# TorbenHellriegel/Speaker-Recognition-x-vectors

Hardware: AMD Instinct MI355X
Metric: x-vector embeddings/sec (300-frame utt) (higher is better)
Workload: dtype f32; 1 GPU; configs[1]: 1xMI355X batch=256 fixed 300-frame x 24-MFCC utterances, fp32 frame-level stack, extract_x_vec layer 6, random-init weights seed 42; build=xvec_hip gfx950 build 527c31bee3f9, batch_per_gpu=256, frames=300

## Files before the change

### speaker-recognition-x-vectors_amd/csrc/tdnn_wino_s3.hip

```cpp
#include "tdnn_wino_rows.h"

namespace xvec {
namespace wino {

constexpr int kS3K = 16;
constexpr int kS3Plane = kPairs * kS3K * 2;
constexpr int kS3Stage = 4 * 3 * kS3Plane;
constexpr int kS3Const = kConst * 4;
constexpr int kS3LdsBytes = 2 * kS3Stage + kS3Const + 2 * kTbl * 4 + 2 * 8;

__device__ __forceinline__ void s3_advance(const TdnnArgs& a, Ctx& cx, const Lane& ln, int* tbl, int64_t* tblh, int n_chunks) {
    if (cx.kc + 1 < n_chunks) {
        ++cx.kc;
    } else {
        const int64_t g_rem = cx.g_end - cx.g_s;
        const int64_t g_next = cx.g_s + (g_rem < 2 ? g_rem : 2);
        if (g_next < cx.g_end) {
            cx.g_s = g_next;
            cx.q0 = g_next * 32;
            cx.lp ^= 1;
            set_rows(a, cx, ln, tbl, tblh);
            cx.kc = 0;
        }
    }
}

struct S3Stage {
    float4 x0, x1, x2, x3;
};

__device__ __forceinline__ void s3_gld(const Ctx& cx, bool grp, S3Stage& s) {
    const int xo0 = grp ? cx.x01 : cx.x00, xo3 = grp ? cx.x31 : cx.x30;
    const int so = cx.kc * (kS3K * 4);
    s.x0 = buf_load16(cx.xrsrc, xo0, so);
    s.x1 = buf_load16(cx.xrsrc, xo0, so + cx.drb);
    s.x2 = buf_load16(cx.xrsrc, xo0, so + 2 * cx.drb);
    s.x3 = buf_load16(cx.xrsrc, xo3, so);
}

__device__ __forceinline__ void s3_vstore(char* B, int st, const S3Stage& s) {
    const float4 v[4] = {
        make_float4(s.x0.x - s.x2.x, s.x0.y - s.x2.y, s.x0.z - s.x2.z, s.x0.w - s.x2.w),
        make_float4(s.x1.x + s.x2.x, s.x1.y + s.x2.y, s.x1.z + s.x2.z, s.x1.w + s.x2.w),
        make_float4(s.x2.x - s.x1.x, s.x2.y - s.x1.y, s.x2.z - s.x1.z, s.x2.w - s.x1.w),
        make_float4(s.x1.x - s.x3.x, s.x1.y - s.x3.y, s.x1.z - s.x3.z, s.x1.w - s.x3.w)};
#pragma unroll
    for (int k = 0; k < 4; ++k) {
        u32x2 hi, mid, lo;
        split3(v[k], hi, mid, lo);
        *reinterpret_cast<u32x2*>(B + (3 * k + 0) * kS3Plane + st) = hi;
        *reinterpret_cast<u32x2*>(B + (3 * k + 1) * kS3Plane + st) = mid;
        *reinterpret_cast<u32x2*>(B + (3 * k + 2) * kS3Plane + st) = lo;
    }
}

__device__ __forceinline__ void s3_uld(__amdgpu_buffer_rsrc_t rsrc, int voff, float4* w, int k, int c, int n_chunks) {
    if (c >= n_chunks) c -= n_chunks;
#pragma unroll
    for (int p = 0; p < 3; ++p) w[p] = buf_load16(rsrc, voff, ((4 * c + k) * 3 + p) * 1024);
}

template <int G>
__device__ __forceinline__ void s3_tile(const TdnnArgs& a, char* lds, int* tbl, int64_t* tblh, Ctx& cx, const Lane& ln,
                                        S3Stage& st, float4 (&w)[4][3], __amdgpu_buffer_rsrc_t ursrc, int n0, int tp,
                                        int n_chunks) {
    const bool grp = (threadIdx.x >> 2) & 1;
    f32x16 acc0_0, acc0_1, acc1_0, acc1_1, acc2_0, acc2_1, acc3_0, acc3_1;
#pragma unroll
    for (int e = 0; e < 16; ++e) {
        acc0_0[e] = 0.f; acc1_0[e] = 0.f; acc2_0[e] = 0.f; acc3_0[e] = 0.f;
        acc0_1[e] = 0.f; acc1_1[e] = 0.f; acc2_1[e] = 0.f; acc3_1[e] = 0.f;
    }
    for (int it = 0; it < n_chunks; ++it) {
        const char* S = lds + (it & 1) * kS3Stage;
        char* Sn = lds + ((it & 1) ^ 1) * kS3Stage;
        s3_vstore(Sn, ln.st_off, st);
        s3_advance(a, cx, ln, tbl, tblh, n_chunks);
        s3_gld(cx, grp, st);
#define WS3_PRODUCT(K_)                                                                                        \
        {                                                                                                      \
            float4 xf0[3], xf1[3];                                                                             \
            _Pragma("unroll") for (int pl = 0; pl < 3; ++pl) {                                                 \
                xf0[pl] = *reinterpret_cast<const float4*>(S + (3 * K_ + pl) * kS3Plane + ln.a_rd);            \
                if constexpr (G > 1)                                                                           \
                    xf1[pl] = *reinterpret_cast<const float4*>(S + (3 * K_ + pl) * kS3Plane + 32 * 32 + ln.a_rd); \
            }                                                                                                  \
            s3_mfma6(acc##K_##_0, xf0, w[K_]);                                                                 \
            if constexpr (G > 1) s3_mfma6(acc##K_##_1, xf1, w[K_]);                                            \
            s3_uld(ursrc, ln.b_rd, w[K_], K_, it + 1, n_chunks);                                               \
        }
        WS3_PRODUCT(0) WS3_PRODUCT(1) WS3_PRODUCT(2) WS3_PRODUCT(3)
#undef WS3_PRODUCT
        __syncthreads();
    }

    epilogue<G>(a, reinterpret_cast<const float*>(lds + 2 * kS3Stage), tbl, tblh, ln, n0, tp, acc0_0, acc1_0, acc2_0, acc3_0, acc0_1,
                acc1_1, acc2_1, acc3_1);
}

__global__ __launch_bounds__(256, 2) void tdnn_wino_s3_kernel(const TdnnArgs a) {
    extern __shared__ __attribute__((aligned(16))) char lds[];
    float* cst = reinterpret_cast<float*>(lds + 2 * kS3Stage);
    int* tbl = reinterpret_cast<int*>(cst + kConst);
    int64_t* tblh = reinterpret_cast<int64_t*>(tbl + 2 * kTbl);
    Ctx cx;
    Lane ln;
    const int n0 = block_setup(a, 3, cx, ln);
    const int n_chunks = 2 * a.cpt;
    const int64_t g_begin = cx.g_s, g_end = cx.g_end;
    const int tid = threadIdx.x, lane = tid & 63, wave = ln.wave;
    ln.st_off = (ln.r0 + 32 * ((tid >> 2) & 1)) * (kS3K * 2) + (tid & 3) * 8;
    ln.a_rd = ln.r * (kS3K * 2) + ln.h * 16;
    ln.b_rd = lane * 16;
    ln.sw = 0;
    const int64_t ct = n0 / 32 + wave;
    const __amdgpu_buffer_rsrc_t ursrc = make_rsrc(static_cast<const char*>(a.Wf) + ct * (int64_t)n_chunks * 12288);

    stream_start(a, n0, cst, tbl, tblh, cx, ln);

    const bool grp = (tid >> 2) & 1;
    S3Stage st;
    float4 w[4][3];
    s3_gld(cx, grp, st);
#pragma unroll
    for (int k = 0; k < 4; ++k) s3_uld(ursrc, ln.b_rd, w[k], k, 0, n_chunks);
    s3_vstore(lds, ln.st_off, st);
    s3_advance(a, cx, ln, tbl, tblh, n_chunks);
    s3_gld(cx, grp, st);
    __syncthreads();

    int64_t g = g_begin;
    int tp = 0;
    for (; g + 2 <= g_end; g += 2, tp ^= 1) s3_tile<2>(a, lds, tbl, tblh, cx, ln, st, w, ursrc, n0, tp, n_chunks);
    if (g < g_end) s3_tile<1>(a, lds, tbl, tblh, cx, ln, st, w, ursrc, n0, tp, n_chunks);
}

}

bool tdnn_wino_s3_applicable(const TdnnGeom& g, int ldx) {
    return tdnn_wino_applicable(g, ldx) && (g.kpt_pad / wino::kS3K) % 2 == 0;
}

hipError_t launch_tdnn_wino_s3(const TdnnArgs& a, hipStream_t s) {
    if (a.groups_total <= 0 || a.blocks_per_col <= 0 || a.blocks_per_col > a.groups_total || a.tap_rows < 1 || a.cpt < 1 ||
        a.Wf == nullptr || (a.out_map.offsets == nullptr && a.p_fixed < 1))
        return hipErrorInvalidValue;
    const int grid = a.blocks_per_col * a.n_tiles;
    wino::tdnn_wino_s3_kernel<<<dim3(grid), dim3(256), wino::kS3LdsBytes, s>>>(a);
    return hipGetLastError();
}

}
```

Measured before the change: 151,400 embeddings/s.

## Software-pipeline S3 Winograd K-loop with interleaved LDS reads and swizzled LDS layout

Restructures the S3 Winograd TDNN inner loop so the MFMAs for each product are interleaved with LDS fragment reads for the next product and with weight buffer loads, using scheduling barriers. The next chunk's first fragments are prefetched across the __syncthreads. It also introduces an XOR-swizzled LDS address map for staging stores and fragment reads, aimed at avoiding bank conflicts. The intent is to hide LDS and global latency behind MFMA work, at the cost of more live registers and more complex control, including an extra barrier when n_chunks is 2.

```diff
diff --git a/profiles/diag/kloop_outline.py b/profiles/diag/kloop_outline.py
--- /dev/null
+++ b/profiles/diag/kloop_outline.py
@@ -0,0 +1,71 @@
+#!/usr/bin/env python3
+import re
+import sys
+
+KINDS = (("mfma", r"v_mfma_"), ("buffer_load", r"buffer_load_"), ("buffer_store", r"buffer_store_"), ("ds_read", r"ds_read"),
+         ("ds_write", r"ds_write"), ("s_barrier", r"s_barrier"), ("v_mov64", r"v_mov_b64|v_pk_mov_b32"),
+         ("branch", r"s_cbranch|s_branch"))
+
+
+def blocks(asm, kernel):
+    out, cur, inside = [], None, False
+    for line in asm.splitlines():
+        s = line.strip()
+        m = re.match(r"^([A-Za-z_.$][\w.$]*):", s)
+        if m:
+            lab = m.group(1)
+            if not lab.startswith(".L"):
+                inside = kernel in lab
+            if inside:
+                cur = (lab, [])
+                out.append(cur)
+            continue
+        if inside and cur is not None and s and not s.startswith((".", ";")):
+            cur[1].append(s.split(";")[0].strip())
+            if s.startswith("s_endpgm"):
+                inside = False
+    return out
+
+
+def kind_of(ins):
+    if ins.startswith("s_waitcnt"):
+        return ins
+    for k, pat in KINDS:
+        if re.match(pat, ins):
+            return k
+    return None
+
+
+def outline(instrs):
+    runs = []
+    for ins in instrs:
+        k = kind_of(ins)
+        if k is None:
+            continue
+        if runs and runs[-1][0] == k and not k.startswith("s_waitcnt"):
+            runs[-1][1] += 1
+        else:
+            runs.append([k, 1])
+    return [k if n == 1 else f"{k} x{n}" for k, n in runs]
+
+
+def main():
+    kernel = sys.argv[1]
+    min_mfma = int(sys.argv[2]) if len(sys.argv) > 2 else 12
+    asm = sys.stdin.read()
+    for lab, ins in blocks(asm, kernel):
+        if sum(1 for i in ins if i.startswith("v_mfma_")) < min_mfma:
+            continue
+        print(f"{lab}:  ({len(ins)} instructions)")
+        line = "   "
+        for item in outline(ins):
+            if len(line) + len(item) > 118:
+                print(line)
+                line = "   "
+            line += " " + item + " |"
+        print(line)
+        print()
+
+
+if __name__ == "__main__":
+    main()
diff --git a/speaker-recognition-x-vectors_amd/csrc/tdnn_wino_s3.hip b/speaker-recognition-x-vectors_amd/csrc/tdnn_wino_s3.hip
--- a/speaker-recognition-x-vectors_amd/csrc/tdnn_wino_s3.hip
+++ b/speaker-recognition-x-vectors_amd/csrc/tdnn_wino_s3.hip
@@ -1,11 +1,10 @@
 #include "tdnn_wino_rows.h"
+#include "wino_s3_lds_map.h"
 
 namespace xvec {
 namespace wino {
 
-constexpr int kS3K = 16;
-constexpr int kS3Plane = kPairs * kS3K * 2;
-constexpr int kS3Stage = 4 * 3 * kS3Plane;
+static_assert(kS3Pairs == kPairs, "wino_s3_lds_map.h: kS3K, kS3Plane, kS3Stage and the image of a (product, plane) block");
 constexpr int kS3Const = kConst * 4;
 constexpr int kS3LdsBytes = 2 * kS3Stage + kS3Const + 2 * kTbl * 4 + 2 * 8;
 
@@ -54,16 +53,54 @@
     }
 }
 
-__device__ __forceinline__ void s3_uld(__amdgpu_buffer_rsrc_t rsrc, int voff, float4* w, int k, int c, int n_chunks) {
-    if (c >= n_chunks) c -= n_chunks;
-#pragma unroll
-    for (int p = 0; p < 3; ++p) w[p] = buf_load16(rsrc, voff, ((4 * c + k) * 3 + p) * 1024);
-}
+struct S3U {
+    float4 w00, w01, w02, w10, w11, w12, w20, w21, w22, w30, w31, w32;
+};
+struct S3Frag {
+    float4 a0, a1, a2, b0, b1, b2;
+};
+
+#define WS3_MF(acc_, x_, w_) \
+    acc_ = __builtin_amdgcn_mfma_f32_32x32x16_bf16(__builtin_bit_cast(bf16x8, x_), __builtin_bit_cast(bf16x8, w_), acc_, 0, 0, 0);
+#define WS3_RD(dst_, B_, kn_, pl_, g_) \
+    dst_ = *reinterpret_cast<const float4*>((B_) + (3 * (kn_) + (pl_)) * kS3Plane + ((g_) ? a_rd1 : ln.a_rd));
+#define WS3_ULD(K_)                                                                   \
+    {                                                                                 \
+        int c_ = it + 1;                                                              \
+        if (c_ >= n_chunks) c_ -= n_chunks;                                           \
+        u.w##K_##0 = buf_load16(ursrc, ln.b_rd, ((4 * c_ + K_) * 3 + 0) * 1024);      \
+        u.w##K_##1 = buf_load16(ursrc, ln.b_rd, ((4 * c_ + K_) * 3 + 1) * 1024);      \
+        u.w##K_##2 = buf_load16(ursrc, ln.b_rd, ((4 * c_ + K_) * 3 + 2) * 1024);      \
+    }
+#define WS3_PRODUCT2(K_, NB_, kn_, BAR_)                                                                   \
+    {                                                                                                      \
+        WS3_MF(acc##K_##_0, f.a2, u.w##K_##0) WS3_RD(f.b2, S, K_, 2, 1) SB();                              \
+        WS3_MF(acc##K_##_0, f.a1, u.w##K_##1) WS3_RD(f.b1, S, K_, 1, 1) SB();                              \
+        WS3_MF(acc##K_##_0, f.a0, u.w##K_##2) WS3_RD(f.b0, S, K_, 0, 1) SB();                              \
+        WS3_MF(acc##K_##_0, f.a1, u.w##K_##0) WS3_MF(acc##K_##_0, f.a0, u.w##K_##1) WS3_MF(acc##K_##_0, f.a0, u.w##K_##0) SB(); \
+        BAR_                                                                                               \
+        WS3_MF(acc##K_##_1, f.b2, u.w##K_##0) WS3_RD(f.a2, NB_, kn_, 2, 0) SB();                           \
+        WS3_MF(acc##K_##_1, f.b1, u.w##K_##1) WS3_RD(f.a1, NB_, kn_, 1, 0) SB();                           \
+        WS3_MF(acc##K_##_1, f.b0, u.w##K_##2) WS3_RD(f.a0, NB_, kn_, 0, 0) SB();                           \
+        WS3_MF(acc##K_##_1, f.b1, u.w##K_##0) WS3_MF(acc##K_##_1, f.b0, u.w##K_##1) WS3_MF(acc##K_##_1, f.b0, u.w##K_##0) SB(); \
+        WS3_ULD(K_)                                                                                        \
+        SB();                                                                                              \
+    }
+#define WS3_PRODUCT1(K_, C_, N_, NB_, kn_, BAR_)                                                           \
+    {                                                                                                      \
+        BAR_                                                                                               \
+        WS3_MF(acc##K_##_0, f.C_##2, u.w##K_##0) WS3_RD(f.N_##2, NB_, kn_, 2, 0) SB();                     \
+        WS3_MF(acc##K_##_0, f.C_##1, u.w##K_##1) WS3_RD(f.N_##1, NB_, kn_, 1, 0) SB();                     \
+        WS3_MF(acc##K_##_0, f.C_##0, u.w##K_##2) WS3_RD(f.N_##0, NB_, kn_, 0, 0) SB();                     \
+        WS3_MF(acc##K_##_0, f.C_##1, u.w##K_##0) WS3_MF(acc##K_##_0, f.C_##0, u.w##K_##1) WS3_MF(acc##K_##_0, f.C_##0, u.w##K_##0) SB(); \
+        WS3_ULD(K_)                                                                                        \
+        SB();                                                                                              \
+    }
 
 template <int G>
 __device__ __forceinline__ void s3_tile(const TdnnArgs& a, char* lds, int* tbl, int64_t* tblh, Ctx& cx, const Lane& ln,
-                                        S3Stage& st, float4 (&w)[4][3], __amdgpu_buffer_rsrc_t ursrc, int n0, int tp,
-                                        int n_chunks) {
+                                        int a_rd1, S3Stage& st, S3U& u, S3Frag& f, __amdgpu_buffer_rsrc_t ursrc, int n0,
+                                        int tp, int n_chunks) {
     const bool grp = (threadIdx.x >> 2) & 1;
     f32x16 acc0_0, acc0_1, acc1_0, acc1_1, acc2_0, acc2_1, acc3_0, acc3_1;
 #pragma unroll
@@ -77,25 +114,23 @@
         s3_vstore(Sn, ln.st_off, st);
         s3_advance(a, cx, ln, tbl, tblh, n_chunks);
         s3_gld(cx, grp, st);
-#define WS3_PRODUCT(K_)                                                                                        \
-        {                                                                                                      \
-            float4 xf0[3], xf1[3];                                                                             \
-            _Pragma("unroll") for (int pl = 0; pl < 3; ++pl) {                                                 \
-                xf0[pl] = *reinterpret_cast<const float4*>(S + (3 * K_ + pl) * kS3Plane + ln.a_rd);            \
-                if constexpr (G > 1)                                                                           \
-                    xf1[pl] = *reinterpret_cast<const float4*>(S + (3 * K_ + pl) * kS3Plane + 32 * 32 + ln.a_rd); \
-            }                                                                                                  \
-            s3_mfma6(acc##K_##_0, xf0, w[K_]);                                                                 \
-            if constexpr (G > 1) s3_mfma6(acc##K_##_1, xf1, w[K_]);                                            \
-            s3_uld(ursrc, ln.b_rd, w[K_], K_, it + 1, n_chunks);                                               \
+        SB();
+        if constexpr (G > 1) {
+            WS3_PRODUCT2(0, S, 1, )
+            WS3_PRODUCT2(1, S, 2, )
+            WS3_PRODUCT2(2, S, 3, )
+            WS3_PRODUCT2(3, Sn, 0, __syncthreads(); SB();)
+        } else {
+            WS3_PRODUCT1(0, a, b, S, 1, )
+            WS3_PRODUCT1(1, b, a, S, 2, )
+            WS3_PRODUCT1(2, a, b, S, 3, )
+            WS3_PRODUCT1(3, b, a, Sn, 0, __syncthreads(); SB();)
         }
-        WS3_PRODUCT(0) WS3_PRODUCT(1) WS3_PRODUCT(2) WS3_PRODUCT(3)
-#undef WS3_PRODUCT
-        __syncthreads();
     }
 
     epilogue<G>(a, reinterpret_cast<const float*>(lds + 2 * kS3Stage), tbl, tblh, ln, n0, tp, acc0_0, acc1_0, acc2_0, acc3_0, acc0_1,
                 acc1_1, acc2_1, acc3_1);
+    if (n_chunks == 2) __syncthreads();
 }
 
 __global__ __launch_bounds__(256, 2) void tdnn_wino_s3_kernel(const TdnnArgs a) {
@@ -109,10 +144,11 @@
     const int n_chunks = 2 * a.cpt;
     const int64_t g_begin = cx.g_s, g_end = cx.g_end;
     const int tid = threadIdx.x, lane = tid & 63, wave = ln.wave;
-    ln.st_off = (ln.r0 + 32 * ((tid >> 2) & 1)) * (kS3K * 2) + (tid & 3) * 8;
-    ln.a_rd = ln.r * (kS3K * 2) + ln.h * 16;
+    ln.st_off = s3_st_off(tid);
+    ln.a_rd = s3_a_rd(lane, 0);
+    const int a_rd1 = s3_a_rd(lane, 1);
+    ln.sw = 0;
     ln.b_rd = lane * 16;
-    ln.sw = 0;
     const int64_t ct = n0 / 32 + wave;
     const __amdgpu_buffer_rsrc_t ursrc = make_rsrc(static_cast<const char*>(a.Wf) + ct * (int64_t)n_chunks * 12288);
 
@@ -120,20 +156,31 @@
 
     const bool grp = (tid >> 2) & 1;
     S3Stage st;
-    float4 w[4][3];
+    S3U u;
+    S3Frag f;
     s3_gld(cx, grp, st);
-#pragma unroll
-    for (int k = 0; k < 4; ++k) s3_uld(ursrc, ln.b_rd, w[k], k, 0, n_chunks);
     s3_vstore(lds, ln.st_off, st);
     s3_advance(a, cx, ln, tbl, tblh, n_chunks);
     s3_gld(cx, grp, st);
+    SB();
+    {
+        const int it = -1;
+        WS3_ULD(0) WS3_ULD(1) WS3_ULD(2) WS3_ULD(3)
+    }
+    SB();
     __syncthreads();
+    WS3_RD(f.a2, lds, 0, 2, 0) WS3_RD(f.a1, lds, 0, 1, 0) WS3_RD(f.a0, lds, 0, 0, 0)
 
     int64_t g = g_begin;
     int tp = 0;
-    for (; g + 2 <= g_end; g += 2, tp ^= 1) s3_tile<2>(a, lds, tbl, tblh, cx, ln, st, w, ursrc, n0, tp, n_chunks);
-    if (g < g_end) s3_tile<1>(a, lds, tbl, tblh, cx, ln, st, w, ursrc, n0, tp, n_chunks);
-}
+    for (; g + 2 <= g_end; g += 2, tp ^= 1) s3_tile<2>(a, lds, tbl, tblh, cx, ln, a_rd1, st, u, f, ursrc, n0, tp, n_chunks);
+    if (g < g_end) s3_tile<1>(a, lds, tbl, tblh, cx, ln, a_rd1, st, u, f, ursrc, n0, tp, n_chunks);
+}
+#undef WS3_PRODUCT2
+#undef WS3_PRODUCT1
+#undef WS3_ULD
+#undef WS3_RD
+#undef WS3_MF
 
 }
 
diff --git a/speaker-recognition-x-vectors_amd/csrc/wino_s3_lds_map.h b/speaker-recognition-x-vectors_amd/csrc/wino_s3_lds_map.h
--- /dev/null
+++ b/speaker-recognition-x-vectors_amd/csrc/wino_s3_lds_map.h
@@ -0,0 +1,20 @@
+#pragma once
+
+namespace xvec {
+namespace wino {
+
+constexpr int kS3K = 16;
+constexpr int kS3Pairs = 64;
+constexpr int kS3Plane = kS3Pairs * kS3K * 2;
+constexpr int kS3Stage = 4 * 3 * kS3Plane;
+
+constexpr int s3_lds_off(int p, int kb) {
+    return (p ^ ((p >> 5) << 1)) * (kS3K * 2) + (((kb >> 4) ^ (p >> 3)) & 1) * 16 + (kb & 15);
+}
+
+constexpr int s3_st_off(int tid) { return s3_lds_off((tid >> 3) + 32 * ((tid >> 2) & 1), (tid & 3) * 8); }
+
+constexpr int s3_a_rd(int lane, int g) { return s3_lds_off(32 * g + (lane & 31), 16 * (lane >> 5)); }
+
+}
+}
```

After: 155,900 embeddings/s, median of 6. 1.03x the previous value.
